# SobeyMIL/MVOC

Measured on AMD Instinct MI355X. Metric: UNet3D denoising steps/sec, 16x512^2 frames, inversion+compose, higher is better.
Workload: dtype f16

## Files before the change

### include/mvoc_hip.h

```cpp
#ifndef MVOC_HIP_H
#define MVOC_HIP_H

#include <stddef.h>
#include <stdint.h>

#ifdef __cplusplus
extern "C" {
#endif

#define MVOC_VERSION 100

int mvoc_version(void);
const char* mvoc_last_error(void);

enum { MVOC_A_PLAIN = 0, MVOC_A_CONV3X3 = 1, MVOC_A_TEMPORAL3 = 2 };
enum { MVOC_ACT_NONE = 0, MVOC_ACT_GEGLU = 1, MVOC_ACT_SILU = 2, MVOC_ACT_GELU = 3 };

typedef struct mvoc_gemm_desc {
  const void* a;
  const void* a2;
  const void* w;
  void* out;
  const void* bias;
  const void* rowadd;
  const void* resid;
  int64_t m, n, k;
  int32_t n_store;
  int32_t ldo, ldr, ld_rowadd, rowadd_div;
  int32_t a_mode;
  int32_t lda, lda2;
  int32_t c1;
  int32_t cin;
  int32_t nimg, hout, wout, hsrc, wsrc, stride, upsample, hup, wup;
  int32_t frames, hw;
  int32_t act;
  int32_t tile;
  int32_t split_k;
  void* workspace;
  size_t workspace_bytes;
  const void* ln_rowsum;
  const void* ln_bias;
  float ln_eps;
  int32_t pad_mode;
  const void* ln_stats;
  void* chan_sums;
  void* row_moments;
  int32_t row_moments_ld;
  int32_t concurrency;
  int32_t k_order;
} mvoc_gemm_desc;

int mvoc_gemm_f16(const mvoc_gemm_desc* d, void* stream);
int mvoc_gemm_chan_sums_written(void);
int mvoc_gemm_row_moments_written(void);
int mvoc_row_stats_from_moments_f32(const void* moments, int64_t rows, int32_t ld, int32_t n, int32_t tile_w, float eps,
                                    void* out_stats, void* stream);
size_t mvoc_gemm_workspace_bytes(int64_t m, int64_t n, int64_t k);

typedef struct mvoc_attn_desc {
  const void *q, *k, *v;
  void* out;
  int64_t q_bs, q_ts, k_bs, k_ts, v_bs, v_ts, o_bs, o_ts;
  int32_t nbatch, heads, tq, tk, kv_bdiv;
  int32_t head_dim, causal;
  float scale;
  const void* v2;
  void* out2;
  int32_t pipelined;
} mvoc_attn_desc;

int mvoc_flash_attn_f16(const mvoc_attn_desc* d, void* stream);
typedef struct mvoc_tattn_desc {
  const void *q, *k, *v;
  void* out;
  int64_t q_bs, q_ps, q_ts, k_bs, k_ps, k_ts, v_bs, v_ps, v_ts, o_bs, o_ps, o_ts;
  int32_t nsample, hw, heads, frames;
} mvoc_tattn_desc;
int mvoc_temporal_attn_f16(const mvoc_tattn_desc* d, void* stream);

typedef struct mvoc_xs_desc {
  const void* x;
  const void* wp;
  const void* resid;
  void* out;
  int64_t m;
  int32_t n, k, n_store, ldo, ldr, act, normalize;
  float ln_eps;
  int64_t wp_set_rows;
} mvoc_xs_desc;
int mvoc_xs_linear_f16(const mvoc_xs_desc* d, void* stream);


typedef struct mvoc_tfused_desc {
  const void* x;
  const void* wp;
  const void* ln_rowsum;
  const void* ln_bias;
  void* out;
  int32_t nsample, frames, hw, c, heads;
  float ln_eps;
} mvoc_tfused_desc;
int mvoc_temporal_qkv_attn_f16(const mvoc_tfused_desc* d, void* stream);

typedef struct mvoc_gn_desc {
  const void* x;
  const void* x2;
  const void* gamma;
  const void* beta;
  void* out;
  void* workspace;
  size_t workspace_bytes;
  int32_t nsample, rows_per_sample, c, c1, groups, silu;
  float eps;
  const void* chan_sums;
  const void* chan_sums2;
} mvoc_gn_desc;
size_t mvoc_groupnorm_workspace_bytes(int32_t nsample, int32_t rows_per_sample, int32_t c, int32_t groups);
int mvoc_groupnorm_f16(const mvoc_gn_desc* d, void* stream);
int mvoc_groupnorm_fold_xs_f16(const mvoc_gn_desc* d, const void* w, const void* bias, int32_t n, int32_t k, void* wp_sets,
                               void* stream);

int mvoc_groupnorm_moments_f16(const mvoc_gn_desc* d, void* moments, void* stream);
int mvoc_groupnorm_apply_moments_f16(const mvoc_gn_desc* d, const void* parts, int32_t nparts, void* stream);

int mvoc_row_stats_f16(const void* x, void* stats, int64_t rows, int32_t c, float eps, void* stream);

int mvoc_layernorm_f16(const void* x, const void* gamma, const void* beta, void* out, int64_t rows, int32_t c,
                       float eps, void* stream);

typedef struct mvoc_pnp_desc {
  void* x;
  void* x2;
  const void* masks;
  int64_t chunk_stride, f_stride, p_stride;
  int32_t nobj, frames, height, width, channels, mask_h, mask_w, base_chunk0;
  int32_t ndst;
} mvoc_pnp_desc;
int mvoc_pnp_blend_scatter_tokens(const mvoc_pnp_desc* d, void* stream);
int mvoc_pnp_blend_scatter_nchw(const mvoc_pnp_desc* d, void* stream);
int mvoc_pnp_blend_scatter_tokens_mapped(const mvoc_pnp_desc* d, int32_t nsrc, const int32_t* obj_chunk, void* stream);
int mvoc_pnp_blend_scatter_nchw_mapped(const mvoc_pnp_desc* d, int32_t nsrc, const int32_t* obj_chunk, void* stream);
int mvoc_pnp_blend_scatter_tokens_variants(const mvoc_pnp_desc* d, int32_t nsrc, const int32_t* obj_chunk, int32_t nvar,
                                           void* stream);
int mvoc_pnp_blend_scatter_nchw_variants(const mvoc_pnp_desc* d, int32_t nsrc, const int32_t* obj_chunk, int32_t nvar,
                                         void* stream);

int mvoc_ddim_step_f16(const void* x, const void* v_uncond, const void* v_cond, const float* coef_dev, void* out,
                       int64_t n, void* stream);
int mvoc_latent_fusion_f16(const void* latents, const void* bg, const void* objs, const void* masks, void* out,
                           int32_t nobj, int64_t n, double mix_ratio, int32_t obj_random_noise_fusion, void* stream);
int mvoc_ddim_step_variants_f16(const void* x, const void* v_uncond, const void* v_cond, const float* coef_dev, void* out,
                                int64_t n_per, int32_t nvar, void* stream);
int mvoc_latent_fusion_variants_f16(const void* latents, const void* bg, const void* objs, const void* masks, void* out,
                                    int32_t nobj, int64_t n_per, int32_t nvar, double mix_ratio,
                                    int32_t obj_random_noise_fusion, void* stream);

int mvoc_timestep_embedding_f16(const float* t_dev, int32_t nb, int32_t dim, void* out, void* stream);
int mvoc_act_f16(const void* x, void* out, int64_t n, int32_t act, void* stream);
int mvoc_add_f16(const void* a, const void* b, void* out, int64_t n, void* stream);
int mvoc_conv3x3_small_f16(const void* x, const void* w, const void* bias, void* out, int32_t nimg, int32_t h,
                           int32_t wd, int32_t cin, int32_t cout, int32_t stride, int32_t silu, void* stream);
int mvoc_adaptive_avgpool_f16(const void* x, void* out, int32_t nimg, int32_t h, int32_t w, int32_t c, int32_t oh,
                              int32_t ow, void* stream);
int mvoc_ncfhw_to_tokens_f16(const void* x, void* out, int32_t b, int32_t c, int32_t f, int32_t hw, int32_t ldo,
                             int32_t coff, void* stream);
int mvoc_tokens_to_ncfhw_f16(const void* x, void* out, int32_t b, int32_t c, int32_t f, int32_t hw, int32_t ld,
                             void* stream);
int mvoc_temporal_encoder4_f16(const void* x, const void* params, void* out, int32_t b, int32_t f, int32_t hw,
                               int32_t ldo, int32_t coff, void* stream);

int mvoc_conv1x1_small_f16(const void* x, const void* w, const void* bias, void* out, int64_t rows, int32_t cin,
                           int32_t cout, void* stream);
int mvoc_softmax_rows_f16(void* x, int64_t rows, int32_t cols, void* stream);
int mvoc_gaussian_sample_f16(const void* mean, const void* logvar, const void* noise, void* out, int64_t n, void* stream);
int mvoc_scale_f16(const void* x, void* out, int64_t n, double scale, void* stream);
int mvoc_image_to_tokens_f16(const void* x, void* out, int32_t n, int32_t c, int32_t hw, void* stream);
int mvoc_tokens_to_image_f16(const void* x, void* out, int32_t n, int32_t c, int32_t hw, int32_t ld, void* stream);

int mvoc_mask_resize_u8(const void* in, void* tmp, void* out, int32_t n, int32_t H, int32_t W, int32_t h, int32_t w,
                        const int32_t* bounds_h, const int32_t* kk_h, int32_t ksize_h, const int32_t* bounds_v,
                        const int32_t* kk_v, int32_t ksize_v, void* stream);
int mvoc_mask_finish(const void* v, void* float_mask, void* bool_mask, int64_t n, void* stream);

int mvoc_clip_patches_f16(const void* pixels, void* out, int32_t nimg, int32_t size, int32_t patch, int32_t kpad, void* stream);
int mvoc_clip_embed_f16(const void* table, const int32_t* ids, const void* cls, const void* pos, void* out, int64_t rows,
                        int32_t t, int32_t c, void* stream);

int mvoc_permute_rows_f16(const void* x, void* out, const int64_t* dims4, const int64_t* strides4, int32_t c, void* stream);
int mvoc_comm_unique_id(void* id128);
int mvoc_comm_init(const void* id128, int32_t rank, int32_t world, void** comm);
int mvoc_comm_destroy(void* comm);
int mvoc_allgather_frames(void* comm, const void* send, void* recv, size_t bytes_per_rank, void* stream);
int mvoc_alltoall_frames(void* comm, const void* send, void* recv, size_t bytes_per_peer, void* stream);

enum { MVOC_FAM_GEMM = 0, MVOC_FAM_FLASH = 1, MVOC_FAM_TATTN = 2, MVOC_FAM_GN = 3, MVOC_FAM_LN = 4, MVOC_FAM_PNP = 5,
       MVOC_FAM_MISC = 6, MVOC_FAM_TFUSED = 7, MVOC_FAM_COUNT = 8 };
int mvoc_prof_enable(int on);
int mvoc_prof_collect(double* ms_per_family, int64_t* launches_per_family, double* flops_or_bytes_per_family);
int mvoc_prof_reset(void);
int mvoc_delay_us(int64_t us, void* stream);

#ifdef __cplusplus
}
#endif
#endif
```

### mvoc_amd/_ffi.py

```python
import ctypes as C
import os

import torch

_HERE = os.path.dirname(os.path.abspath(__file__))
LIB_PATH = os.environ.get("MVOC_HIP_LIB") or os.path.join(_HERE, "libmvoc_hip.so")

ABI_VERSION = 100

A_PLAIN, A_CONV3X3, A_TEMPORAL3 = 0, 1, 2
ACT_NONE, ACT_GEGLU, ACT_SILU, ACT_GELU = 0, 1, 2, 3
FAMILIES = ("gemm", "flash_attn", "temporal_attn", "groupnorm", "layernorm", "pnp", "misc", "temporal_fused")

vp, i32, i64, f32, f64, sz = C.c_void_p, C.c_int32, C.c_int64, C.c_float, C.c_double, C.c_size_t


class GemmDesc(C.Structure):
    _fields_ = [("a", vp), ("a2", vp), ("w", vp), ("out", vp), ("bias", vp), ("rowadd", vp), ("resid", vp),
                ("m", i64), ("n", i64), ("k", i64), ("n_store", i32), ("ldo", i32), ("ldr", i32), ("ld_rowadd", i32),
                ("rowadd_div", i32), ("a_mode", i32), ("lda", i32), ("lda2", i32), ("c1", i32), ("cin", i32),
                ("nimg", i32), ("hout", i32), ("wout", i32), ("hsrc", i32), ("wsrc", i32), ("stride", i32),
                ("upsample", i32), ("hup", i32), ("wup", i32), ("frames", i32), ("hw", i32), ("act", i32), ("tile", i32),
                ("split_k", i32), ("workspace", vp), ("workspace_bytes", sz), ("ln_rowsum", vp), ("ln_bias", vp),
                ("ln_eps", f32), ("pad_mode", i32), ("ln_stats", vp), ("chan_sums", vp), ("row_moments", vp),
                ("row_moments_ld", i32), ("concurrency", i32), ("k_order", i32)]


class AttnDesc(C.Structure):
    _fields_ = [("q", vp), ("k", vp), ("v", vp), ("out", vp),
                ("q_bs", i64), ("q_ts", i64), ("k_bs", i64), ("k_ts", i64), ("v_bs", i64), ("v_ts", i64),
                ("o_bs", i64), ("o_ts", i64),
                ("nbatch", i32), ("heads", i32), ("tq", i32), ("tk", i32), ("kv_bdiv", i32),
                ("head_dim", i32), ("causal", i32), ("scale", C.c_float), ("v2", vp), ("out2", vp), ("pipelined", i32)]


class TAttnDesc(C.Structure):
    _fields_ = [("q", vp), ("k", vp), ("v", vp), ("out", vp),
                ("q_bs", i64), ("q_ps", i64), ("q_ts", i64), ("k_bs", i64), ("k_ps", i64), ("k_ts", i64),
                ("v_bs", i64), ("v_ps", i64), ("v_ts", i64), ("o_bs", i64), ("o_ps", i64), ("o_ts", i64),
                ("nsample", i32), ("hw", i32), ("heads", i32), ("frames", i32)]


class GnDesc(C.Structure):
    _fields_ = [("x", vp), ("x2", vp), ("gamma", vp), ("beta", vp), ("out", vp), ("workspace", vp),
                ("workspace_bytes", sz), ("nsample", i32), ("rows_per_sample", i32), ("c", i32), ("c1", i32),
                ("groups", i32), ("silu", i32), ("eps", f32), ("chan_sums", vp), ("chan_sums2", vp)]


class TFusedDesc(C.Structure):
    _fields_ = [("x", vp), ("wp", vp), ("ln_rowsum", vp), ("ln_bias", vp), ("out", vp), ("nsample", i32), ("frames", i32),
                ("hw", i32), ("c", i32), ("heads", i32), ("ln_eps", f32)]


class XsDesc(C.Structure):
    _fields_ = [("x", vp), ("wp", vp), ("resid", vp), ("out", vp), ("m", i64),
                ("n", i32), ("k", i32), ("n_store", i32), ("ldo", i32), ("ldr", i32), ("act", i32), ("normalize", i32),
                ("ln_eps", C.c_float), ("wp_set_rows", i64)]


class PnpDesc(C.Structure):
    _fields_ = [("x", vp), ("x2", vp), ("masks", vp), ("chunk_stride", i64), ("f_stride", i64), ("p_stride", i64),
                ("nobj", i32), ("frames", i32), ("height", i32), ("width", i32), ("channels", i32), ("mask_h", i32),
                ("mask_w", i32), ("base_chunk0", i32), ("ndst", i32)]


SIGNATURES = {
    "mvoc_version": (i32, []),
    "mvoc_last_error": (C.c_char_p, []),
    "mvoc_gemm_f16": (i32, [C.POINTER(GemmDesc), vp]),
    "mvoc_gemm_workspace_bytes": (sz, [i64, i64, i64]),
    "mvoc_gemm_chan_sums_written": (i32, []),
    "mvoc_gemm_row_moments_written": (i32, []),
    "mvoc_row_stats_from_moments_f32": (i32, [vp, i64, i32, i32, i32, f32, vp, vp]),
    "mvoc_flash_attn_f16": (i32, [C.POINTER(AttnDesc), vp]),
    "mvoc_temporal_attn_f16": (i32, [C.POINTER(TAttnDesc), vp]),
    "mvoc_temporal_qkv_attn_f16": (i32, [C.POINTER(TFusedDesc), vp]),
    "mvoc_xs_linear_f16": (i32, [C.POINTER(XsDesc), vp]),
    "mvoc_groupnorm_workspace_bytes": (sz, [i32, i32, i32, i32]),
    "mvoc_groupnorm_f16": (i32, [C.POINTER(GnDesc), vp]),
    "mvoc_groupnorm_fold_xs_f16": (i32, [C.POINTER(GnDesc), vp, vp, i32, i32, vp, vp]),
    "mvoc_groupnorm_moments_f16": (i32, [C.POINTER(GnDesc), vp, vp]),
    "mvoc_groupnorm_apply_moments_f16": (i32, [C.POINTER(GnDesc), vp, i32, vp]),
    "mvoc_layernorm_f16": (i32, [vp, vp, vp, vp, i64, i32, f32, vp]),
    "mvoc_row_stats_f16": (i32, [vp, vp, i64, i32, f32, vp]),
    "mvoc_pnp_blend_scatter_tokens": (i32, [C.POINTER(PnpDesc), vp]),
    "mvoc_pnp_blend_scatter_nchw": (i32, [C.POINTER(PnpDesc), vp]),
    "mvoc_pnp_blend_scatter_tokens_mapped": (i32, [C.POINTER(PnpDesc), i32, C.POINTER(i32), vp]),
    "mvoc_pnp_blend_scatter_nchw_mapped": (i32, [C.POINTER(PnpDesc), i32, C.POINTER(i32), vp]),
    "mvoc_pnp_blend_scatter_tokens_variants": (i32, [C.POINTER(PnpDesc), i32, C.POINTER(i32), i32, vp]),
    "mvoc_pnp_blend_scatter_nchw_variants": (i32, [C.POINTER(PnpDesc), i32, C.POINTER(i32), i32, vp]),
    "mvoc_ddim_step_f16": (i32, [vp, vp, vp, vp, vp, i64, vp]),
    "mvoc_latent_fusion_f16": (i32, [vp, vp, vp, vp, vp, i32, i64, f64, i32, vp]),
    "mvoc_ddim_step_variants_f16": (i32, [vp, vp, vp, vp, vp, i64, i32, vp]),
    "mvoc_latent_fusion_variants_f16": (i32, [vp, vp, vp, vp, vp, i32, i64, i32, f64, i32, vp]),
    "mvoc_timestep_embedding_f16": (i32, [vp, i32, i32, vp, vp]),
    "mvoc_act_f16": (i32, [vp, vp, i64, i32, vp]),
    "mvoc_add_f16": (i32, [vp, vp, vp, i64, vp]),
    "mvoc_conv3x3_small_f16": (i32, [vp, vp, vp, vp, i32, i32, i32, i32, i32, i32, i32, vp]),
    "mvoc_adaptive_avgpool_f16": (i32, [vp, vp, i32, i32, i32, i32, i32, i32, vp]),
    "mvoc_ncfhw_to_tokens_f16": (i32, [vp, vp, i32, i32, i32, i32, i32, i32, vp]),
    "mvoc_tokens_to_ncfhw_f16": (i32, [vp, vp, i32, i32, i32, i32, i32, vp]),
    "mvoc_temporal_encoder4_f16": (i32, [vp, vp, vp, i32, i32, i32, i32, i32, vp]),
    "mvoc_conv1x1_small_f16": (i32, [vp, vp, vp, vp, i64, i32, i32, vp]),
    "mvoc_softmax_rows_f16": (i32, [vp, i64, i32, vp]),
    "mvoc_gaussian_sample_f16": (i32, [vp, vp, vp, vp, i64, vp]),
    "mvoc_scale_f16": (i32, [vp, vp, i64, f64, vp]),
    "mvoc_image_to_tokens_f16": (i32, [vp, vp, i32, i32, i32, vp]),
    "mvoc_tokens_to_image_f16": (i32, [vp, vp, i32, i32, i32, i32, vp]),
    "mvoc_mask_resize_u8": (i32, [vp, vp, vp, i32, i32, i32, i32, i32, vp, vp, i32, vp, vp, i32, vp]),
    "mvoc_mask_finish": (i32, [vp, vp, vp, i64, vp]),
    "mvoc_permute_rows_f16": (i32, [vp, vp, C.POINTER(i64), C.POINTER(i64), i32, vp]),
    "mvoc_clip_patches_f16": (i32, [vp, vp, i32, i32, i32, i32, vp]),
    "mvoc_clip_embed_f16": (i32, [vp, vp, vp, vp, vp, i64, i32, i32, vp]),
    "mvoc_comm_unique_id": (i32, [vp]),
    "mvoc_comm_init": (i32, [vp, i32, i32, C.POINTER(vp)]),
    "mvoc_comm_destroy": (i32, [vp]),
    "mvoc_allgather_frames": (i32, [vp, vp, vp, sz, vp]),
    "mvoc_alltoall_frames": (i32, [vp, vp, vp, sz, vp]),
    "mvoc_prof_enable": (i32, [i32]),
    "mvoc_prof_collect": (i32, [C.POINTER(f64), C.POINTER(i64), C.POINTER(f64)]),
    "mvoc_prof_reset": (i32, []),
    "mvoc_delay_us": (i32, [i64, vp]),
}


def _load():
    if not os.path.exists(LIB_PATH):
        raise ImportError(
            f"{LIB_PATH} is missing: build it with `python -m mvoc_amd.build` (hipcc --offload-arch=gfx950). "
            "mvoc_amd has no CPU / PyTorch fallback path.")
    lib = C.CDLL(LIB_PATH)
    for name, (res, args) in SIGNATURES.items():
        fn = getattr(lib, name)
        fn.restype = res
        fn.argtypes = args
    if lib.mvoc_version() != ABI_VERSION:
        raise ImportError(f"{LIB_PATH} has mvoc_version() {lib.mvoc_version()}, these bindings need {ABI_VERSION}: rebuild it "
                          "with `python -m mvoc_amd.build`")
    return lib


lib = _load()


_DEBUG_SYNC = bool(os.environ.get("MVOC_DEBUG_SYNC"))


def check(rc, what=""):
    if rc != 0:
        raise RuntimeError(f"libmvoc_hip {what} failed ({rc}): {lib.mvoc_last_error().decode()}")
    if _DEBUG_SYNC:
        print(f"[mvoc] {what}", flush=True)
        torch.cuda.synchronize()
```

### mvoc_amd/csrc/attention.hip

```cpp
#include <stdlib.h>

#include "common.h"

namespace {

typedef __fp16 fp16x4_t __attribute__((__vector_size__(4 * sizeof(__fp16))));
template <int D> struct FlashPitch { static constexpr int K = 2 * D + 16, V = D == 64 ? 192 : 320; };

struct AttnArgs {
  const half_t *q, *k, *v;
  half_t* out;
  long q_bs, q_ts, k_bs, k_ts, v_bs, v_ts, o_bs, o_ts;
  int nbatch, heads, tq, tk, kv_bdiv, causal;
  float scale_log2;
  long v2_off, o2_off;
  int qblocks;
};

__device__ __forceinline__ int vt_slot_group(int key) {
  return ((((key >> 5) * 2 + ((key >> 4) & 1)) * 2) + ((key >> 2) & 1));
}
__device__ __forceinline__ int vt_slot_elem(int key) { return ((key >> 3) & 1) * 4 + (key & 3); }

constexpr float FLASH_THR = 8.0f;
// ... 302 lines not shown
#pragma unroll
  for (int e = 0; e < 16; ++e) zero16[e] = 0.f;

  int kfo[4];
#pragma unroll
  for (int s = 0; s < 4; ++s) kfo[s] = r * 128 + (((2 * s + h) ^ ((r >> 1) & 7)) * 16);
  const int vq = (lane & 15) >> 2;
  int vfo[2];
#pragma unroll
  for (int dt = 0; dt < 2; ++dt) vfo[dt] = 8192 + (4 * h + vq) * 128 + (((32 * ((lane >> 4) & 1) + 8 * (lane & 3))) | ((dt ^ ((vq >> 1) & 1)) << 6));

  f3_wait_vm<(NS - 2) * PCS>();
  F3_BAR();
#pragma unroll
  for (int t = 0; t < 2; ++t) {
    sa[t] = zero16;
#pragma unroll
    for (int s = 0; s < 4; ++s) {
      const half8_t kf = *reinterpret_cast<const half8_t*>(smem + kfo[s] + 4096 * t);
      sa[t] = __builtin_amdgcn_mfma_f32_32x32x16_f16(kf, qf[s], sa[t], 0, 0, 0);
    }
  }
  int o_v = 0, o_k = TILE, o_w = (NS - 1) * TILE;

  auto body = [&](f32x16(&cur)[2], f32x16(&nxt)[2], const int t) {
    F3_STAMP(4);
    f3_wait_vm<(NS - 3) * PCS>();
    F3_BAR();
    F3_STAMP(0);
    issue(t + NS - 1, o_w);
    F3_FENCE();
    F3_STAMP(1);
    const char* Kn = smem + o_k;
    const char* Vc = smem + o_v;
    if (__builtin_amdgcn_readfirstlane((t == nt - 1) && (p.tk & 63))) {
#pragma unroll
      for (int tt = 0; tt < 2; ++tt)
#pragma unroll
        for (int e = 0; e < 16; ++e)
          if (t * 64 + 32 * tt + 8 * (e >> 2) + 4 * h + (e & 3) >= p.tk) cur[tt][e] = -INFINITY;
    }
    F3_FENCE();
    half8_t kf[2][4];
#pragma unroll
    for (int s = 0; s < 2; ++s)
#pragma unroll
      for (int tt = 0; tt < 2; ++tt) kf[tt][s] = *reinterpret_cast<const half8_t*>(Kn + kfo[s] + 4096 * tt);
    half8_t pf[2];
    half8_t vf[3][NV][2];
    auto vread = [&](const int f) {
#pragma unroll
      for (int v = 0; v < NV; ++v)
#pragma unroll
        for (int dt = 0; dt < 2; ++dt) {
          const char* va = Vc + 8192 * v + vfo[dt] + (32 * (f >> 1) + 16 * (f & 1)) * 128;
          const fp16x4_t lo = __builtin_amdgcn_ds_read_tr16_b64_v4f16((__attribute__((address_space(3))) fp16x4_t*)va);
          const fp16x4_t hi = __builtin_amdgcn_ds_read_tr16_b64_v4f16((__attribute__((address_space(3))) fp16x4_t*)(va + 8 * 128));
#pragma unroll
          for (int e = 0; e < 4; ++e) {
            vf[f % 3][v][dt][e] = (half_t)lo[e];
            vf[f % 3][v][dt][4 + e] = (half_t)hi[e];
          }
        }
    };
    vread(0);
    F3_FENCE();
    auto smma = [&](const int i) {
      const int tt = i & 1, s_ = i >> 1;
      nxt[tt] = __builtin_amdgcn_mfma_f32_32x32x16_f16(kf[tt][s_], qf[s_], s_ == 0 ? zero16 : nxt[tt], 0, 0, 0);
    };
    auto pvmma = [&](const int f, const int dt) {
#pragma unroll
      for (int v = 0; v < NV; ++v) ot[v][dt] = __builtin_amdgcn_mfma_f32_32x32x16_f16(vf[f % 3][v][dt], pf[f & 1], ot[v][dt], 0, 0, 0);
    };
    float mx = fmaxf(cur[0][0], cur[0][1]);
#pragma unroll
    for (int tt = 0; tt < 2; ++tt)
#pragma unroll
      for (int e = tt ? 0 : 2; e < 16; e += 2) mx = __builtin_fmaxf(__builtin_fmaxf(mx, cur[tt][e]), cur[tt][e + 1]);
    smma(0); smma(1); smma(2);
    if constexpr (NV == 2) smma(3);
    mx = flash_xhalf_max(mx);
    if constexpr (NV == 1) { F3_GRP(6, 0); F3_GRP(6, 0); F3_GRP(6, 0); }
    else { F3_GRP(4, 0); F3_GRP(5, 0); F3_GRP(4, 0); F3_GRP(5, 0); }
    F3_STAMP(2);
    if (__any((mx - mrun) * p.scale_log2 > FLASH_THR)) {
      const float mnew = fmaxf(mrun, mx);
      const float alpha = __builtin_amdgcn_exp2f((mrun - mnew) * p.scale_log2);
      mrun = mnew;
      lrun *= alpha;
#pragma unroll
      for (int v = 0; v < NV; ++v)
#pragma unroll
        for (int dt = 0; dt < 2; ++dt)
#pragma unroll
          for (int e = 0; e < 16; ++e) ot[v][dt][e] *= alpha;
    }
    F3_FENCE();
    const f32x2 sc2 = {p.scale_log2, p.scale_log2}, mc2 = {-mrun * p.scale_log2, -mrun * p.scale_log2};
#pragma unroll
    for (int s = 2; s < 4; ++s)
#pragma unroll
      for (int tt = 0; tt < 2; ++tt) kf[tt][s] = *reinterpret_cast<const half8_t*>(Kn + kfo[s] + 4096 * tt);
#pragma unroll
    for (int f = 0; f < 4; ++f) {
      const int tt = f >> 1, s_ = f & 1;
      if (f < 3) vread(f + 1);
      half8_t& pn = pf[f & 1];
      float x[8];
#pragma unroll
      for (int j = 0; j < 8; j += 2) {
        const f32x2 a = __builtin_elementwise_fma(f32x2{cur[tt][8 * s_ + j], cur[tt][8 * s_ + j + 1]}, sc2, mc2);
        x[j] = __builtin_amdgcn_exp2f(a[0]);
        x[j + 1] = __builtin_amdgcn_exp2f(a[1]);
      }
#pragma unroll
      for (int j = 0; j < 8; ++j) pn[j] = (half_t)x[j];
#pragma unroll
      for (int j = 0; j < 4; ++j) lrun = __builtin_amdgcn_fdot2(half2_t{pn[2 * j], pn[2 * j + 1]}, half2_t{(half_t)1.f, (half_t)1.f}, lrun, false);
      if (f == 0) {
        smma(NV == 1 ? 3 : 4); smma(NV == 1 ? 4 : 5);
        if constexpr (NV == 2) { smma(6); smma(7); } else smma(5);
      } else {
        pvmma(f - 1, 0); pvmma(f - 1, 1);
        if constexpr (NV == 1) { if (f < 3) smma(5 + f); }
      }
    }
    pvmma(3, 0);
    pvmma(3, 1);
    if constexpr (NV == 1) {
      F3_RD(8); F3_GRP(5, 3); F3_GRP(5, 2); F3_GRP(5, 3);
      F3_RD(4); F3_GRP(5, 2); F3_GRP(5, 3); F3_GRP(5, 2);
      F3_RD(4); F3_GRP(5, 3); F3_GRP(5, 2); F3_GRP(5, 3);
      F3_GRP(5, 2); F3_GRP(5, 3); F3_GRP(5, 2); F3_GRP(5, 2);
    } else {
      F3_RD(12); F3_GRP(3, 2); F3_GRP(3, 2); F3_GRP(3, 2); F3_GRP(3, 2);
      F3_RD(8); F3_GRP(3, 2); F3_GRP(3, 2); F3_GRP(3, 2); F3_GRP(3, 2);
      F3_RD(8); F3_GRP(3, 2); F3_GRP(3, 2); F3_GRP(3, 2); F3_GRP(3, 2);
      F3_GRP(3, 2); F3_GRP(3, 2); F3_GRP(3, 2); F3_GRP(3, 2);
      F3_GRP(3, 0); F3_GRP(3, 0); F3_GRP(3, 0); F3_GRP(3, 0);
    }
    F3_FENCE();
    F3_STAMP(3);
    const int o_ = o_v; o_v = o_k;
    o_k = o_k + TILE == NS * TILE ? 0 : o_k + TILE;
    o_w = o_;
  };
#pragma unroll 1
  for (int t = 0;; t += 2) {
    body(sa, sb, t);
    if (t + 1 >= nt) break;
    body(sb, sa, t + 1);
    if (t + 2 >= nt) break;
  }
  f3_wait_vm<0>();
#ifdef MVOC_F3_STAMPS
  if (blockIdx.x == 0 && tid == 0) {
    unsigned long long t1_, r1_;
    asm volatile("s_memtime %0\n\ts_memrealtime %1\n\ts_waitcnt lgkmcnt(0)" : "=s"(t1_), "=s"(r1_)::"memory");
    for (int i = 0; i < 5; ++i) f3_dbg[i] = f3_acc[i];
    f3_dbg[5] = t1_ - f3_t0;
    f3_dbg[7] = r1_ - f3_r0;
    f3_dbg[6] = (unsigned long long)nt;
  }
#endif

  const float ltot = lrun + __shfl_xor(lrun, 32);
  const float inv = 1.0f / ltot;
  if (q0 + r < p.tq) {
#pragma unroll
    for (int v = 0; v < NV; ++v) {
      half_t* op = p.out + v * p.o2_off + (long)b * p.o_bs + (long)(q0 + r) * p.o_ts + head * D;
#pragma unroll
      for (int dt = 0; dt < 2; ++dt)
#pragma unroll
        for (int q = 0; q < 4; ++q) {
          half4_t o;
#pragma unroll
          for (int e = 0; e < 4; ++e) o[e] = (half_t)(ot[v][dt][q * 4 + e] * inv);
          *reinterpret_cast<half4_t*>(op + 32 * dt + 8 * q + 4 * h) = o;
        }
    }
  }
}
#undef F3_BAR
#undef F3_FENCE
#undef F3_GRP
#undef F3_RD
#undef F3_STAMP

struct TAttnArgs {
  const half_t *q, *k, *v;
  half_t* out;
  long q_bs, q_ps, q_ts, k_bs, k_ps, k_ts, v_bs, v_ps, v_ts, o_bs, o_ps, o_ts;
  int nsample, hw, heads, frames;
  int logf, logp, pgroups;
  long ntask;
  float scale_log2;
};

constexpr int TVPITCH = 64;

__global__ __launch_bounds__(256) void tattn_kernel(const TAttnArgs p) {
  __shared__ __attribute__((aligned(16))) char smem[4 * 64 * TVPITCH];
  const int tid = threadIdx.x, lane = tid & 63, wave = tid >> 6;
  const int r = lane & 31, h = lane >> 5;
  char* Vs = smem + wave * 64 * TVPITCH;
  const int F = p.frames, logf = p.logf, P = 1 << p.logp;
  const long task = (long)blockIdx.x * 4 + wave;
  const bool active = task < p.ntask;
  const long tk = active ? task : p.ntask - 1;
  const int head = (int)(tk % p.heads);
  const long bp = tk / p.heads;
  const long smp = bp / p.pgroups, px0 = (bp % p.pgroups) << p.logp;
  const half8_t zero8 = {0, 0, 0, 0, 0, 0, 0, 0};
  auto row_px = [&](int row) { return (long)(P > 1 ? row >> logf : 0); };
  auto row_fr = [&](int row) { return P > 1 ? row & (F - 1) : row; };
  auto row_ok = [&](int row) { return (P > 1 || row < F) && px0 + row_px(row) < p.hw; };

  const half_t* qb = p.q + smp * p.q_bs + px0 * p.q_ps + head * 64;
  const half_t* kb = p.k + smp * p.k_bs + px0 * p.k_ps + head * 64;
  const half_t* vb = p.v + smp * p.v_bs + px0 * p.v_ps + head * 64;

#pragma unroll
  for (int i = 0; i < 4; ++i) {
    const int c = lane + 64 * i;
    const int key = c >> 3, dc = c & 7;
    half8_t vr = zero8;
    if (row_ok(key)) vr = *reinterpret_cast<const half8_t*>(vb + row_px(key) * p.v_ps + (long)row_fr(key) * p.v_ts + dc * 8);
    const int g = (((key >> 4) & 1) * 2) + ((key >> 2) & 1), j = vt_slot_elem(key);
#pragma unroll
    for (int e = 0; e < 8; ++e) {
      const int d = dc * 8 + e;
      *reinterpret_cast<half_t*>(Vs + d * TVPITCH + ((g ^ ((d >> 3) & 3)) * 16) + j * 2) = vr[e];
    }
  }
  f32x16 st;
#pragma unroll
  for (int e = 0; e < 16; ++e) st[e] = 0.f;
  const bool rok = row_ok(r);
  const long koff = row_px(r) * p.k_ps + (long)row_fr(r) * p.k_ts, qoff = row_px(r) * p.q_ps + (long)row_fr(r) * p.q_ts;
#pragma unroll
  for (int s = 0; s < 4; ++s) {
    half8_t kf = zero8, qf = zero8;
    if (rok) {
      kf = *reinterpret_cast<const half8_t*>(kb + koff + 16 * s + 8 * h);
      qf = *reinterpret_cast<const half8_t*>(qb + qoff + 16 * s + 8 * h);
    }
    st = __builtin_amdgcn_mfma_f32_32x32x16_f16(kf, qf, st, 0, 0, 0);
  }
  float mx = -INFINITY;
#pragma unroll
  for (int e = 0; e < 16; ++e) {
    const int key = 8 * (e >> 2) + 4 * h + (e & 3);
    const bool ok = P > 1 ? (key >> logf) == (r >> logf) : key < F;
    const float sv = ok ? st[e] * p.scale_log2 : -INFINITY;
    st[e] = sv;
    mx = fmaxf(mx, sv);
  }
  mx = fmaxf(mx, __shfl_xor(mx, 32));
  float ps = 0.f;
#pragma unroll
  for (int e = 0; e < 16; ++e) {
    const float pv = __builtin_amdgcn_exp2f(st[e] - mx);
    st[e] = pv;
    ps += pv;
  }
  ps += __shfl_xor(ps, 32);
  const float inv = 1.0f / ps;

  __syncthreads();
  f32x16 ot[2];
#pragma unroll
  for (int dt = 0; dt < 2; ++dt)
#pragma unroll
    for (int e = 0; e < 16; ++e) ot[dt][e] = 0.f;
#pragma unroll
  for (int s = 0; s < 2; ++s) {
    half8_t pf;
#pragma unroll
    for (int j = 0; j < 8; ++j) pf[j] = (half_t)st[8 * s + j];
    const int g = s * 2 + h;
#pragma unroll
    for (int dt = 0; dt < 2; ++dt) {
      const int d = 32 * dt + r;
      const half8_t vf = *reinterpret_cast<const half8_t*>(Vs + d * TVPITCH + ((g ^ ((d >> 3) & 3)) * 16));
      ot[dt] = __builtin_amdgcn_mfma_f32_32x32x16_f16(vf, pf, ot[dt], 0, 0, 0);
    }
  }
  if (active && rok) {
    half_t* op = p.out + smp * p.o_bs + (px0 + row_px(r)) * p.o_ps + (long)row_fr(r) * p.o_ts + head * 64;
#pragma unroll
    for (int dt = 0; dt < 2; ++dt)
#pragma unroll
      for (int q = 0; q < 4; ++q) {
        half4_t o;
#pragma unroll
        for (int e = 0; e < 4; ++e) o[e] = (half_t)(ot[dt][q * 4 + e] * inv);
        *reinterpret_cast<half4_t*>(op + 32 * dt + 8 * q + 4 * h) = o;
      }
  }
}

}

static const int g_f3_env = getenv("MVOC_FLASH3") ? atoi(getenv("MVOC_FLASH3")) : -1;

extern "C" int mvoc_flash_attn_f16(const mvoc_attn_desc* d, void* stream) {
  MVOC_REQUIRE(d && d->q && d->k && d->v && d->out, -1, "flash_attn: null operand");
  MVOC_REQUIRE(d->nbatch > 0 && d->heads > 0 && d->tq > 0 && d->tk > 0, -1, "flash_attn: empty problem");
  MVOC_REQUIRE(d->nbatch <= 65535 && d->heads <= 65535, -2, "flash_attn: grid too large");
  MVOC_REQUIRE(d->q_ts % 8 == 0 && d->k_ts % 8 == 0 && d->v_ts % 8 == 0 && d->o_ts % 4 == 0, -2,
               "flash_attn: row strides must keep 16-byte alignment");
  AttnArgs a;
  a.q = (const half_t*)d->q; a.k = (const half_t*)d->k; a.v = (const half_t*)d->v; a.out = (half_t*)d->out;
  a.q_bs = d->q_bs; a.q_ts = d->q_ts; a.k_bs = d->k_bs; a.k_ts = d->k_ts; a.v_bs = d->v_bs; a.v_ts = d->v_ts;
  a.o_bs = d->o_bs; a.o_ts = d->o_ts;
  a.nbatch = d->nbatch; a.heads = d->heads; a.tq = d->tq; a.tk = d->tk; a.kv_bdiv = d->kv_bdiv > 0 ? d->kv_bdiv : 1;
  const int hd = d->head_dim > 0 ? d->head_dim : 64;
  MVOC_REQUIRE(hd == 64 || hd == 96, -2, "flash_attn: head_dim (%d) must be 64 or 96", hd);
  MVOC_REQUIRE(!d->causal || d->tq == d->tk, -2, "flash_attn: the causal form is self-attention (tq == tk)");
  a.causal = d->causal;
  a.scale_log2 = (d->scale > 0.f ? d->scale : (hd == 64 ? 0.125f : 1.0f / sqrtf((float)hd))) * 1.4426950408889634f;
  hipStream_t s = (hipStream_t)stream;
  MvocProfScope prof(MVOC_FAM_FLASH, s, (d->v2 ? 2.0 : 1.0) * 4.0 * d->nbatch * d->heads * (double)d->tq * d->tk * hd);
  a.qblocks = (d->tq + 127) / 128;
  const long nblk = (long)a.qblocks * d->heads * d->nbatch;
  MVOC_REQUIRE(nblk < 0x7fffffffL, -2, "flash_attn: grid too large");
  dim3 grid((unsigned)nblk);
  a.v2_off = a.o2_off = 0;
  MVOC_REQUIRE(d->pipelined >= 0 && d->pipelined <= 2, -1, "flash_attn: pipelined must be 0 (by key count), 1 (never) or 2 (wherever it applies)");
  const int f3_mode = d->pipelined ? d->pipelined - 1 : g_f3_env;
  const bool pipelined = hd == 64 && !d->causal && (f3_mode >= 0 ? f3_mode != 0 : d->tk >= 2048);
  if (d->v2) {
    MVOC_REQUIRE(d->out2 && hd == 64, -2, "flash_attn: the paired form needs out2 and head_dim 64");
    a.v2_off = (const half_t*)d->v2 - a.v;
    a.o2_off = (half_t*)d->out2 - a.out;
    MVOC_REQUIRE(a.v2_off % 8 == 0 && a.o2_off % 4 == 0, -2, "flash_attn: v2 / out2 must keep 16-byte alignment");
    if (pipelined) hipLaunchKernelGGL((flash3_kernel<2>), grid, dim3(256), 0, s, a);
    else hipLaunchKernelGGL((flash_kernel<64, 2>), grid, dim3(256), 0, s, a);
  } else if (hd == 64) {
    if (pipelined) hipLaunchKernelGGL((flash3_kernel<1>), grid, dim3(256), 0, s, a);
    else hipLaunchKernelGGL((flash_kernel<64, 1>), grid, dim3(256), 0, s, a);
  } else {
    hipLaunchKernelGGL((flash_kernel<96, 1>), grid, dim3(256), 0, s, a);
  }
  return mvoc_check_launch("flash_kernel");
}

#ifdef MVOC_F3_STAMPS
extern "C" int mvoc_f3_stamps_read(unsigned long long* host8) {
  return hipMemcpyFromSymbol(host8, HIP_SYMBOL(f3_dbg), sizeof(unsigned long long) * 8) == hipSuccess ? 0 : -1;
}
#endif

extern "C" int mvoc_temporal_attn_f16(const mvoc_tattn_desc* d, void* stream) {
  MVOC_REQUIRE(d && d->q && d->k && d->v && d->out, -1, "temporal_attn: null operand");
  MVOC_REQUIRE(d->nsample > 0 && d->hw > 0 && d->heads > 0, -1, "temporal_attn: empty problem");
  MVOC_REQUIRE(d->frames >= 1 && d->frames <= 32, -2, "temporal_attn: frames (%d) must be in [1, 32]", d->frames);
  MVOC_REQUIRE(d->q_ts % 8 == 0 && d->k_ts % 8 == 0 && d->v_ts % 8 == 0 && d->o_ts % 4 == 0 && d->q_ps % 8 == 0 &&
                   d->k_ps % 8 == 0 && d->v_ps % 8 == 0 && d->o_ps % 4 == 0,
               -2, "temporal_attn: strides must keep 16-byte alignment");
  TAttnArgs a;
  a.q = (const half_t*)d->q; a.k = (const half_t*)d->k; a.v = (const half_t*)d->v; a.out = (half_t*)d->out;
  a.q_bs = d->q_bs; a.q_ps = d->q_ps; a.q_ts = d->q_ts; a.k_bs = d->k_bs; a.k_ps = d->k_ps; a.k_ts = d->k_ts;
  a.v_bs = d->v_bs; a.v_ps = d->v_ps; a.v_ts = d->v_ts; a.o_bs = d->o_bs; a.o_ps = d->o_ps; a.o_ts = d->o_ts;
  a.nsample = d->nsample; a.hw = d->hw; a.heads = d->heads; a.frames = d->frames;
  a.logf = d->frames == 8 ? 3 : d->frames == 16 ? 4 : 5;
  a.logp = d->frames == 8 ? 2 : d->frames == 16 ? 1 : 0;
  a.pgroups = (d->hw + (1 << a.logp) - 1) >> a.logp;
  a.ntask = (long)d->nsample * a.pgroups * d->heads;
  a.scale_log2 = 0.125f * 1.4426950408889634f;
  const long nblk = (a.ntask + 3) / 4;
  MVOC_REQUIRE(nblk < 0x7fffffffL, -2, "temporal_attn: grid too large");
  hipStream_t s = (hipStream_t)stream;
  MvocProfScope prof(MVOC_FAM_TATTN, s, 4.0 * (double)d->nsample * d->hw * d->heads * d->frames * 64 * 2);
  hipLaunchKernelGGL(tattn_kernel, dim3((unsigned)nblk), dim3(256), 0, s, a);
  return mvoc_check_launch("tattn_kernel");
}
```

Baseline: 21.56.

## Add KV-resident cross-attention kernel and streaming temporal attention kernel

Adds a kernel for short-key attention (at most 192 keys, e.g. text cross-attention). It loads the whole K/V set for a head into LDS once and loops persistent waves over many 32-query tiles, prefetching the next Q tile. Adds a streaming temporal-attention kernel for 8 or 16 frames that processes several tasks per wave with software-prefetched Q/K/V loads and per-wave LDS staging of V. Both are picked by new dispatch helpers under alignment and size conditions, falling back to the old kernels otherwise. The cost is more code paths and dynamic LDS sizing that may limit occupancy.

```diff
diff --git a/include/mvoc_hip.h b/include/mvoc_hip.h
--- a/include/mvoc_hip.h
+++ b/include/mvoc_hip.h
@@ -70,6 +70,10 @@
 } mvoc_attn_desc;
 
 int mvoc_flash_attn_f16(const mvoc_attn_desc* d, void* stream);
+#define MVOC_ATTN_KERNEL_PHASE 0
+#define MVOC_ATTN_KERNEL_PIPELINED 1
+#define MVOC_ATTN_KERNEL_RESIDENT 2
+int mvoc_flash_attn_kernel_for(const mvoc_attn_desc* d);
 typedef struct mvoc_tattn_desc {
   const void *q, *k, *v;
   void* out;
@@ -77,6 +81,9 @@
   int32_t nsample, hw, heads, frames;
 } mvoc_tattn_desc;
 int mvoc_temporal_attn_f16(const mvoc_tattn_desc* d, void* stream);
+#define MVOC_TATTN_KERNEL_TILE 0
+#define MVOC_TATTN_KERNEL_STREAM 1
+int mvoc_temporal_attn_kernel_for(const mvoc_tattn_desc* d);
 
 typedef struct mvoc_xs_desc {
   const void* x;
diff --git a/mvoc_amd/_ffi.py b/mvoc_amd/_ffi.py
--- a/mvoc_amd/_ffi.py
+++ b/mvoc_amd/_ffi.py
@@ -10,6 +10,8 @@
 
 A_PLAIN, A_CONV3X3, A_TEMPORAL3 = 0, 1, 2
 ACT_NONE, ACT_GEGLU, ACT_SILU, ACT_GELU = 0, 1, 2, 3
+ATTN_KERNEL_PHASE, ATTN_KERNEL_PIPELINED, ATTN_KERNEL_RESIDENT = 0, 1, 2
+TATTN_KERNEL_TILE, TATTN_KERNEL_STREAM = 0, 1
 FAMILIES = ("gemm", "flash_attn", "temporal_attn", "groupnorm", "layernorm", "pnp", "misc", "temporal_fused")
 
 vp, i32, i64, f32, f64, sz = C.c_void_p, C.c_int32, C.c_int64, C.c_float, C.c_double, C.c_size_t
@@ -74,6 +76,8 @@
     "mvoc_row_stats_from_moments_f32": (i32, [vp, i64, i32, i32, i32, f32, vp, vp]),
     "mvoc_flash_attn_f16": (i32, [C.POINTER(AttnDesc), vp]),
     "mvoc_temporal_attn_f16": (i32, [C.POINTER(TAttnDesc), vp]),
+    "mvoc_flash_attn_kernel_for": (i32, [C.POINTER(AttnDesc)]),
+    "mvoc_temporal_attn_kernel_for": (i32, [C.POINTER(TAttnDesc)]),
     "mvoc_temporal_qkv_attn_f16": (i32, [C.POINTER(TFusedDesc), vp]),
     "mvoc_xs_linear_f16": (i32, [C.POINTER(XsDesc), vp]),
     "mvoc_groupnorm_workspace_bytes": (sz, [i32, i32, i32, i32]),
diff --git a/mvoc_amd/csrc/attention.hip b/mvoc_amd/csrc/attention.hip
--- a/mvoc_amd/csrc/attention.hip
+++ b/mvoc_amd/csrc/attention.hip
@@ -628,9 +628,351 @@
   }
 }
 
+__device__ __forceinline__ void store_rows16(half_t* op, const f32x16 (&ot)[2], const float inv, const bool live) {
+#pragma unroll
+  for (int dt = 0; dt < 2; ++dt) {
+    unsigned pk[4][2];
+#pragma unroll
+    for (int q = 0; q < 4; ++q)
+#pragma unroll
+      for (int w = 0; w < 2; ++w) {
+        const half2_t v2 = {(half_t)(ot[dt][q * 4 + 2 * w] * inv), (half_t)(ot[dt][q * 4 + 2 * w + 1] * inv)};
+        pk[q][w] = __builtin_bit_cast(unsigned, v2);
+      }
+#pragma unroll
+    for (int qq = 0; qq < 4; qq += 2)
+#pragma unroll
+      for (int w = 0; w < 2; ++w) {
+        const auto sw = __builtin_amdgcn_permlane32_swap(pk[qq][w], pk[qq + 1][w], false, false);
+        pk[qq][w] = sw[0];
+        pk[qq + 1][w] = sw[1];
+      }
+    if (live) {
+#pragma unroll
+      for (int j = 0; j < 2; ++j) {
+        const uint4 v = {pk[2 * j][0], pk[2 * j][1], pk[2 * j + 1][0], pk[2 * j + 1][1]};
+        *reinterpret_cast<uint4*>(op + 32 * dt + 16 * j) = v;
+      }
+    }
+  }
+}
+
+struct KvResArgs {
+  AttnArgs a;
+  int tpi, wpb, chunks;
+};
+
+template <int NW>
+__global__ __launch_bounds__(NW * 64, 4) void kvres_kernel(const KvResArgs pp) {
+  const AttnArgs& p = pp.a;
+  constexpr int D = 64, KPITCH = FlashPitch<D>::K, VPITCH = FlashPitch<D>::V, ND = 4, NT = 2, NTH = NW * 64;
+  constexpr int NCH = 192 * 8 / NTH;
+  extern __shared__ __attribute__((aligned(16))) char kvres_smem[];
+  const int ntiles = (p.tk + 63) / 64;
+  char* Ks = kvres_smem;
+  char* Vs = kvres_smem + ntiles * 64 * KPITCH;
+  const int tid = threadIdx.x, lane = tid & 63;
+  const int wave = __builtin_amdgcn_readfirstlane(tid >> 6);
+  const int r = lane & 31, h = lane >> 5;
+  const unsigned logical = xcd_remap(blockIdx.x, gridDim.x);
+  const unsigned chunk = logical % (unsigned)pp.chunks, hb_ = logical / (unsigned)pp.chunks;
+  const int head = (int)(hb_ % (unsigned)p.heads), g = (int)(hb_ / (unsigned)p.heads);
+  const int b0 = g * p.kv_bdiv;
+  const int ntile_g = min(p.kv_bdiv, p.nbatch - b0) * pp.tpi;
+  const int tend = min(((int)chunk + 1) * pp.wpb, ntile_g);
+  int t = (int)chunk * pp.wpb + wave;
+
+  const half_t* qp = p.q + head * D + 8 * h;
+  auto loadq = [&](const int tt, half8_t(&qf)[ND], int& b, int& q0) {
+    const int img = tt / pp.tpi;
+    b = b0 + img;
+    q0 = (tt - img * pp.tpi) * 32;
+    const half_t* qrow = qp + (long)b * p.q_bs + (long)min(q0 + r, p.tq - 1) * p.q_ts;
+#pragma unroll
+    for (int s = 0; s < ND; ++s) qf[s] = *reinterpret_cast<const half8_t*>(qrow + 16 * s);
+  };
+  half8_t qn[ND];
+  int bn = 0, q0n = 0;
+  if (t < tend) loadq(t, qn, bn, q0n);
+
+  {
+    const char* kb = reinterpret_cast<const char*>(p.k + (long)g * p.k_bs + head * D);
+    const char* vb = reinterpret_cast<const char*>(p.v + (long)g * p.v_bs + head * D);
+    const unsigned k_rb = (unsigned)p.k_ts * 2u, v_rb = (unsigned)p.v_ts * 2u;
+    const int nch = ntiles * 64 * 8;
+    half8_t kreg[NCH], vreg[NCH];
+#pragma unroll
+    for (int i = 0; i < NCH; ++i) {
+      const int c = tid + i * NTH;
+      if (i * NTH < nch) {
+        const unsigned row = (unsigned)min(c >> 3, p.tk - 1), col = (unsigned)(c & 7) * 16u;
+        kreg[i] = *reinterpret_cast<const half8_t*>(kb + (size_t)row * k_rb + col);
+        vreg[i] = *reinterpret_cast<const half8_t*>(vb + (size_t)row * v_rb + col);
+      }
+    }
+#pragma unroll
+    for (int i = 0; i < NCH; ++i) {
+      const int c = tid + i * NTH;
+      if (i * NTH < nch) {
+        *reinterpret_cast<half8_t*>(Ks + (c >> 3) * KPITCH + (c & 7) * 16) = kreg[i];
+        *reinterpret_cast<half8_t*>(Vs + (c >> 3) * VPITCH + (c & 7) * 16) = vreg[i];
+      }
+    }
+  }
+  __syncthreads();
+
+  while (t < tend) {
+    half8_t qf[ND];
+#pragma unroll
+    for (int s = 0; s < ND; ++s) qf[s] = qn[s];
+    const int b = bn, q0 = q0n;
+    t += NW;
+    if (t < tend) loadq(t, qn, bn, q0n);
+
+    f32x16 ot[NT];
+#pragma unroll
+    for (int dt = 0; dt < NT; ++dt)
+#pragma unroll
+      for (int e = 0; e < 16; ++e) ot[dt][e] = 0.f;
+    float mrun = -INFINITY, lrun = 0.f;
+#pragma unroll 1
+    for (int kt = 0; kt < ntiles; ++kt) {
+      const char* Kt = Ks + kt * 64 * KPITCH;
+      const char* Vt = Vs + kt * 64 * VPITCH;
+      f32x16 st[2];
+#pragma unroll
+      for (int tt = 0; tt < 2; ++tt) {
+#pragma unroll
+        for (int e = 0; e < 16; ++e) st[tt][e] = 0.f;
+#pragma unroll
+        for (int s = 0; s < ND; ++s) {
+          const half8_t kf = *reinterpret_cast<const half8_t*>(Kt + (32 * tt + r) * KPITCH + (16 * s + 8 * h) * 2);
+          st[tt] = __builtin_amdgcn_mfma_f32_32x32x16_f16(kf, qf[s], st[tt], 0, 0, 0);
+        }
+      }
+      if (__builtin_amdgcn_readfirstlane((kt == ntiles - 1) && (p.tk & 63))) {
+#pragma unroll
+        for (int tt = 0; tt < 2; ++tt)
+#pragma unroll
+          for (int e = 0; e < 16; ++e)
+            if (kt * 64 + 32 * tt + 8 * (e >> 2) + 4 * h + (e & 3) >= p.tk) st[tt][e] = -INFINITY;
+      }
+      float mx = st[0][0];
+#pragma unroll
+      for (int tt = 0; tt < 2; ++tt)
+#pragma unroll
+        for (int e = 0; e < 16; ++e) mx = fmaxf(mx, st[tt][e]);
+      mx = flash_xhalf_max(mx);
+      if (__any((mx - mrun) * p.scale_log2 > FLASH_THR)) {
+        const float mnew = fmaxf(mrun, mx);
+        const float alpha = __builtin_amdgcn_exp2f((mrun - mnew) * p.scale_log2);
+        mrun = mnew;
+        lrun *= alpha;
+#pragma unroll
+        for (int dt = 0; dt < NT; ++dt)
+#pragma unroll
+          for (int e = 0; e < 16; ++e) ot[dt][e] *= alpha;
+      }
+      const f32x2 sc2 = {p.scale_log2, p.scale_log2}, mc2 = {-mrun * p.scale_log2, -mrun * p.scale_log2};
+#pragma unroll
+      for (int tt = 0; tt < 2; ++tt)
+#pragma unroll
+        for (int e = 0; e < 16; e += 2) {
+          const f32x2 a = __builtin_elementwise_fma(f32x2{st[tt][e], st[tt][e + 1]}, sc2, mc2);
+          st[tt][e] = __builtin_amdgcn_exp2f(a[0]);
+          st[tt][e + 1] = __builtin_amdgcn_exp2f(a[1]);
+        }
+#pragma unroll
+      for (int tt = 0; tt < 2; ++tt)
+#pragma unroll
+        for (int s = 0; s < 2; ++s) {
+          half8_t pf;
+#pragma unroll
+          for (int j = 0; j < 8; ++j) pf[j] = (half_t)st[tt][8 * s + j];
+#pragma unroll
+          for (int j = 0; j < 4; ++j) lrun = __builtin_amdgcn_fdot2(half2_t{pf[2 * j], pf[2 * j + 1]}, half2_t{(half_t)1.f, (half_t)1.f}, lrun, false);
+          const int krow = 32 * tt + 16 * s + 4 * h + ((lane & 15) >> 2);
+#pragma unroll
+          for (int dt = 0; dt < NT; ++dt) {
+            const char* va = Vt + krow * VPITCH + (32 * dt + 16 * ((lane >> 4) & 1) + 4 * (lane & 3)) * 2;
+            const fp16x4_t lo = __builtin_amdgcn_ds_read_tr16_b64_v4f16((__attribute__((address_space(3))) fp16x4_t*)va);
+            const fp16x4_t hi = __builtin_amdgcn_ds_read_tr16_b64_v4f16((__attribute__((address_space(3))) fp16x4_t*)(va + 8 * VPITCH));
+            half8_t vf;
+#pragma unroll
+            for (int e = 0; e < 4; ++e) {
+              vf[e] = (half_t)lo[e];
+              vf[4 + e] = (half_t)hi[e];
+            }
+            ot[dt] = __builtin_amdgcn_mfma_f32_32x32x16_f16(vf, pf, ot[dt], 0, 0, 0);
+          }
+        }
+    }
+    const float ltot = lrun + __shfl_xor(lrun, 32);
+    const float inv = 1.0f / ltot;
+    half_t* op = p.out + (long)b * p.o_bs + (long)min(q0 + r, p.tq - 1) * p.o_ts + head * D + 8 * h;
+    store_rows16(op, ot, inv, q0 + r < p.tq);
+  }
+}
+
+struct TStreamArgs {
+  TAttnArgs a;
+  int nit;
+};
+
+__global__ __launch_bounds__(256) void tstream_kernel(const TStreamArgs pp) {
+  const TAttnArgs& p = pp.a;
+  constexpr int VP = FlashPitch<64>::V;
+  __shared__ __attribute__((aligned(16))) char smem[4 * 32 * VP];
+  const int tid = threadIdx.x, lane = tid & 63;
+  const int wave = __builtin_amdgcn_readfirstlane(tid >> 6);
+  const int r = lane & 31, h = lane >> 5;
+  char* Vs = smem + wave * 32 * VP;
+  const int F = p.frames, logf = p.logf;
+  const half8_t zero8 = {0, 0, 0, 0, 0, 0, 0, 0};
+  const int rpx = r >> logf, rfr = r & (F - 1);
+  const unsigned qo = (unsigned)((rpx * p.q_ps + rfr * p.q_ts) * 2 + 16 * h);
+  const unsigned ko = (unsigned)((rpx * p.k_ps + rfr * p.k_ts) * 2 + 16 * h);
+  const unsigned oo = (unsigned)((rpx * p.o_ps + rfr * p.o_ts) * 2 + 16 * h);
+  const unsigned qo0 = (unsigned)(rfr * p.q_ts * 2 + 16 * h), ko0 = (unsigned)(rfr * p.k_ts * 2 + 16 * h);
+  unsigned vo[4], vo0[4];
+  int vpx[4];
+#pragma unroll
+  for (int i = 0; i < 4; ++i) {
+    const int key = (lane >> 3) + 8 * i;
+    vpx[i] = key >> logf;
+    vo[i] = (unsigned)((vpx[i] * p.v_ps + (key & (F - 1)) * p.v_ts) * 2 + (lane & 7) * 16);
+    vo0[i] = (unsigned)((key & (F - 1)) * p.v_ts * 2 + (lane & 7) * 16);
+  }
+  const unsigned vw = (unsigned)((lane >> 3) * VP + (lane & 7) * 16);
+  const int vkrow = 4 * h + ((lane & 15) >> 2);
+  const unsigned vr = (unsigned)(vkrow * VP + (16 * ((lane >> 4) & 1) + 4 * (lane & 3)) * 2);
+
+  const int tend = (int)min(((long)blockIdx.x + 1) * 4 * pp.nit, p.ntask);
+  int task = (int)blockIdx.x * 4 * pp.nit + wave;
+  auto gload = [&](const int tk, half8_t(&qf)[4], half8_t(&kf)[4], half8_t(&vf)[4], const char*& ob, int& live) {
+    const unsigned bp = __builtin_amdgcn_readfirstlane((unsigned)tk / (unsigned)p.heads);
+    const unsigned head = __builtin_amdgcn_readfirstlane((unsigned)tk - bp * (unsigned)p.heads);
+    const unsigned smp = __builtin_amdgcn_readfirstlane(bp / (unsigned)p.pgroups);
+    const int px0 = __builtin_amdgcn_readfirstlane((int)((bp - smp * (unsigned)p.pgroups) << p.logp));
+    live = p.hw - px0;
+    const char* qb = reinterpret_cast<const char*>(p.q + (long)smp * p.q_bs + (long)px0 * p.q_ps + head * 64);
+    const char* kb = reinterpret_cast<const char*>(p.k + (long)smp * p.k_bs + (long)px0 * p.k_ps + head * 64);
+    const char* vb = reinterpret_cast<const char*>(p.v + (long)smp * p.v_bs + (long)px0 * p.v_ps + head * 64);
+    ob = reinterpret_cast<const char*>(p.out + (long)smp * p.o_bs + (long)px0 * p.o_ps + head * 64);
+    const unsigned qa = rpx < live ? qo : qo0, ka = rpx < live ? ko : ko0;
+#pragma unroll
+    for (int s = 0; s < 4; ++s) {
+      kf[s] = *reinterpret_cast<const half8_t*>(kb + ka + 32 * s);
+      qf[s] = *reinterpret_cast<const half8_t*>(qb + qa + 32 * s);
+    }
+#pragma unroll
+    for (int i = 0; i < 4; ++i) vf[i] = *reinterpret_cast<const half8_t*>(vb + (vpx[i] < live ? vo[i] : vo0[i]));
+  };
+  half8_t qn[4], kn[4], vn[4];
+  const char* obn = nullptr;
+  int liven = 0;
+  if (task < tend) gload(task, qn, kn, vn, obn, liven);
+  while (task < tend) {
+    half8_t qf[4], kf[4], vc[4];
+#pragma unroll
+    for (int s = 0; s < 4; ++s) {
+      qf[s] = qn[s];
+      kf[s] = kn[s];
+      vc[s] = vn[s];
+    }
+    const char* ob = obn;
+    const int live = liven;
+    if (live < (32 >> logf)) {
+#pragma unroll
+      for (int s = 0; s < 4; ++s) {
+        if (rpx >= live) qf[s] = kf[s] = zero8;
+        if (vpx[s] >= live) vc[s] = zero8;
+      }
+    }
+    task += 4;
+    if (task < tend) gload(task, qn, kn, vn, obn, liven);
+
+    __builtin_amdgcn_fence(__ATOMIC_RELEASE, "wavefront");
+#pragma unroll
+    for (int i = 0; i < 4; ++i) *reinterpret_cast<half8_t*>(Vs + vw + i * 8 * VP) = vc[i];
+    __builtin_amdgcn_fence(__ATOMIC_SEQ_CST, "wavefront");
+
+    f32x16 st;
+#pragma unroll
+    for (int e = 0; e < 16; ++e) st[e] = 0.f;
+#pragma unroll
+    for (int s = 0; s < 4; ++s) st = __builtin_amdgcn_mfma_f32_32x32x16_f16(kf[s], qf[s], st, 0, 0, 0);
+    float mx = -INFINITY;
+#pragma unroll
+    for (int e = 0; e < 16; ++e) {
+      const int key = 8 * (e >> 2) + 4 * h + (e & 3);
+      const bool ok = (key >> logf) == (r >> logf);
+      const float sv = ok ? st[e] * p.scale_log2 : -INFINITY;
+      st[e] = sv;
+      mx = fmaxf(mx, sv);
+    }
+    mx = fmaxf(mx, __shfl_xor(mx, 32));
+    float ps = 0.f;
+#pragma unroll
+    for (int e = 0; e < 16; ++e) {
+      const float pv = __builtin_amdgcn_exp2f(st[e] - mx);
+      st[e] = pv;
+      ps += pv;
+    }
+    ps += __shfl_xor(ps, 32);
+    const float inv = 1.0f / ps;
+
+    f32x16 ot[2];
+#pragma unroll
+    for (int dt = 0; dt < 2; ++dt)
+#pragma unroll
+      for (int e = 0; e < 16; ++e) ot[dt][e] = 0.f;
+#pragma unroll
+    for (int s = 0; s < 2; ++s) {
+      half8_t pf;
+#pragma unroll
+      for (int j = 0; j < 8; ++j) pf[j] = (half_t)st[8 * s + j];
+#pragma unroll
+      for (int dt = 0; dt < 2; ++dt) {
+        const char* va = Vs + vr + s * 16 * VP + dt * 64;
+        const fp16x4_t lo = __builtin_amdgcn_ds_read_tr16_b64_v4f16((__attribute__((address_space(3))) fp16x4_t*)va);
+        const fp16x4_t hi = __builtin_amdgcn_ds_read_tr16_b64_v4f16((__attribute__((address_space(3))) fp16x4_t*)(va + 8 * VP));
+        half8_t vf;
+#pragma unroll
+        for (int e = 0; e < 4; ++e) {
+          vf[e] = (half_t)lo[e];
+          vf[4 + e] = (half_t)hi[e];
+        }
+        ot[dt] = __builtin_amdgcn_mfma_f32_32x32x16_f16(vf, pf, ot[dt], 0, 0, 0);
+      }
+    }
+    store_rows16(reinterpret_cast<half_t*>(const_cast<char*>(ob) + oo), ot, inv, rpx < live);
+  }
+}
+
 }
 
 static const int g_f3_env = getenv("MVOC_FLASH3") ? atoi(getenv("MVOC_FLASH3")) : -1;
+constexpr int KVRES_MAX_KEYS = 192, KVRES_MIN_QUERIES = 32;
+#ifndef KVRES_ROUNDS
+#define KVRES_ROUNDS 2
+#endif
+#ifndef TSTREAM_SLOTS
+#define TSTREAM_SLOTS 512
+#endif
+
+extern "C" int mvoc_flash_attn_kernel_for(const mvoc_attn_desc* d) {
+  MVOC_REQUIRE(d, -1, "flash_attn_kernel_for: null descriptor");
+  MVOC_REQUIRE(d->pipelined >= 0 && d->pipelined <= 2, -1, "flash_attn: pipelined must be 0 (by key count), 1 (never) or 2 (wherever it applies)");
+  const int hd = d->head_dim > 0 ? d->head_dim : 64;
+  const int f3_mode = d->pipelined ? d->pipelined - 1 : g_f3_env;
+  if (hd == 64 && !d->causal && (f3_mode >= 0 ? f3_mode != 0 : d->tk >= 2048)) return MVOC_ATTN_KERNEL_PIPELINED;
+  const long kvb = d->kv_bdiv > 0 ? d->kv_bdiv : 1;
+  if (f3_mode < 0 && hd == 64 && !d->causal && !d->v2 && d->tk <= KVRES_MAX_KEYS && kvb * d->tq >= KVRES_MIN_QUERIES && d->o_ts % 8 == 0 &&
+      d->o_bs % 8 == 0 && ((uintptr_t)d->out & 15) == 0)
+    return MVOC_ATTN_KERNEL_RESIDENT;
+  return MVOC_ATTN_KERNEL_PHASE;
+}
 
 extern "C" int mvoc_flash_attn_f16(const mvoc_attn_desc* d, void* stream) {
   MVOC_REQUIRE(d && d->q && d->k && d->v && d->out, -1, "flash_attn: null operand");
@@ -655,9 +997,25 @@
   MVOC_REQUIRE(nblk < 0x7fffffffL, -2, "flash_attn: grid too large");
   dim3 grid((unsigned)nblk);
   a.v2_off = a.o2_off = 0;
-  MVOC_REQUIRE(d->pipelined >= 0 && d->pipelined <= 2, -1, "flash_attn: pipelined must be 0 (by key count), 1 (never) or 2 (wherever it applies)");
-  const int f3_mode = d->pipelined ? d->pipelined - 1 : g_f3_env;
-  const bool pipelined = hd == 64 && !d->causal && (f3_mode >= 0 ? f3_mode != 0 : d->tk >= 2048);
+  const int kernel = mvoc_flash_attn_kernel_for(d);
+  if (kernel < 0) return kernel;
+  const bool pipelined = kernel == MVOC_ATTN_KERNEL_PIPELINED;
+  if (kernel == MVOC_ATTN_KERNEL_RESIDENT) {
+    KvResArgs r;
+    r.a = a;
+    r.tpi = (d->tq + 31) / 32;
+    const long ngroup = (d->nbatch + a.kv_bdiv - 1) / a.kv_bdiv, per_gh = (long)min(a.kv_bdiv, d->nbatch) * r.tpi;
+    const int nw = per_gh >= 16 ? 8 : 4;
+    const long want = (ngroup * d->heads * per_gh + 512L * KVRES_ROUNDS - 1) / (512L * KVRES_ROUNDS);
+    r.wpb = (int)min(max((want + nw - 1) / nw, 1L), 8L) * nw;
+    r.chunks = (int)((per_gh + r.wpb - 1) / r.wpb);
+    const long nb = ngroup * d->heads * r.chunks;
+    MVOC_REQUIRE(nb < 0x7fffffffL, -2, "flash_attn: grid too large");
+    const size_t lds = (size_t)((d->tk + 63) / 64) * 64 * (FlashPitch<64>::K + FlashPitch<64>::V);
+    if (nw == 8) hipLaunchKernelGGL((kvres_kernel<8>), dim3((unsigned)nb), dim3(512), lds, s, r);
+    else hipLaunchKernelGGL((kvres_kernel<4>), dim3((unsigned)nb), dim3(256), lds, s, r);
+    return mvoc_check_launch("kvres_kernel");
+  }
   if (d->v2) {
     MVOC_REQUIRE(d->out2 && hd == 64, -2, "flash_attn: the paired form needs out2 and head_dim 64");
     a.v2_off = (const half_t*)d->v2 - a.v;
@@ -679,6 +1037,19 @@
   return hipMemcpyFromSymbol(host8, HIP_SYMBOL(f3_dbg), sizeof(unsigned long long) * 8) == hipSuccess ? 0 : -1;
 }
 #endif
+
+extern "C" int mvoc_temporal_attn_kernel_for(const mvoc_tattn_desc* d) {
+  MVOC_REQUIRE(d, -1, "temporal_attn_kernel_for: null descriptor");
+  if (d->frames != 8 && d->frames != 16) return MVOC_TATTN_KERNEL_TILE;
+  if (d->o_ps % 8 || d->o_ts % 8 || d->o_bs % 8 || ((uintptr_t)d->out & 15)) return MVOC_TATTN_KERNEL_TILE;
+  const int64_t px = 32 / d->frames - 1, fr = d->frames - 1;
+  for (const int64_t span : {px * d->q_ps + fr * d->q_ts, px * d->k_ps + fr * d->k_ts, px * d->v_ps + fr * d->v_ts, px * d->o_ps + fr * d->o_ts})
+    if (span < 0 || span >= (1LL << 30)) return MVOC_TATTN_KERNEL_TILE;
+  for (const int64_t st : {d->q_ps, d->q_ts, d->k_ps, d->k_ts, d->v_ps, d->v_ts, d->o_ps, d->o_ts})
+    if (st < 0) return MVOC_TATTN_KERNEL_TILE;
+  if ((int64_t)d->nsample * d->hw * d->heads >= (1LL << 31)) return MVOC_TATTN_KERNEL_TILE;
+  return MVOC_TATTN_KERNEL_STREAM;
+}
 
 extern "C" int mvoc_temporal_attn_f16(const mvoc_tattn_desc* d, void* stream) {
   MVOC_REQUIRE(d && d->q && d->k && d->v && d->out, -1, "temporal_attn: null operand");
@@ -701,6 +1072,15 @@
   MVOC_REQUIRE(nblk < 0x7fffffffL, -2, "temporal_attn: grid too large");
   hipStream_t s = (hipStream_t)stream;
   MvocProfScope prof(MVOC_FAM_TATTN, s, 4.0 * (double)d->nsample * d->hw * d->heads * d->frames * 64 * 2);
+  const int kernel = mvoc_temporal_attn_kernel_for(d);
+  if (kernel < 0) return kernel;
+  if (kernel == MVOC_TATTN_KERNEL_STREAM) {
+    TStreamArgs t;
+    t.a = a;
+    t.nit = (int)min(max(nblk / TSTREAM_SLOTS, 1L), 8L);
+    hipLaunchKernelGGL(tstream_kernel, dim3((unsigned)((nblk + t.nit - 1) / t.nit)), dim3(256), 0, s, t);
+    return mvoc_check_launch("tstream_kernel");
+  }
   hipLaunchKernelGGL(tattn_kernel, dim3((unsigned)nblk), dim3(256), 0, s, a);
   return mvoc_check_launch("tattn_kernel");
 }
```

Result: no change. 21.73 (median of 6 runs) (+0.8%).
